# liuxinren456852/HiDeGS

Measured on AMD Instinct MI355X. Metric: binning-stage iters/sec at 2M Gaussians, 1920x1080 (scan + tile sort + ranges, the built part of the fwd+bwd iteration; the rasterizer fwd/bwd is not built: headline_metric, status), higher is better.
Workload: dtype u64/u32 (binning), f32 (distCUDA2, exchange, masked Adam)

## Files before the change

hidegs_amd/csrc/common.h:

```cpp
#pragma once
#include <hip/hip_runtime.h>
#include <stddef.h>
#include <stdint.h>

#include <string>

#include "../../include/hidegs.h"

namespace hidegs {

void set_error(const std::string& msg);
const std::string& last_error();

inline int fail(int code, const std::string& msg)
{
    set_error(msg);
    return code;
}

inline hipStream_t as_stream(void* s) { return reinterpret_cast<hipStream_t>(s); }

int check_launch(const char* stage, hipStream_t stream, int debug);

bool debug_enabled();

int queue_error(hipStream_t stream, int clear, uint32_t* flags);

uint32_t* async_error_slot(hipStream_t stream);
int take_async_error(const char* what, hipStream_t stream);
uint32_t take_async_bits(hipStream_t stream);

size_t sort_u64_scratch(long long n);
int sort_pairs_u64(void* scratch, size_t bytes, const uint64_t* ki, uint64_t* ko, const uint32_t* vi, uint32_t* vo,
                   long long n, int b, int e, hipStream_t s);

constexpr size_t kAlign = 256;
inline size_t align_up(size_t n) { return (n + kAlign - 1) & ~(kAlign - 1); }

struct Carver {
    char* base;
    size_t used = 0;
    explicit Carver(void* b) : base(static_cast<char*>(b)) {}
    template <typename T>
    T* take(size_t count)
    {
        T* p = reinterpret_cast<T*>(base ? base + used : nullptr);
        used += align_up(count * sizeof(T));
        return p;
    }
};

constexpr int kWave = 64;

__device__ __forceinline__ int lane_id() { return __lane_id(); }

__device__ __forceinline__ int xcd_swizzle(int b, int nb)
{
    const int per = nb / 8, rem = nb % 8, x = b % 8, k = b / 8;
    return (x < rem) ? x * (per + 1) + k : rem * (per + 1) + (x - rem) * per + k;
}

template <typename T>
__device__ __forceinline__ T wave_shfl_xor(T v, int m)
{
    return __shfl_xor(v, m, kWave);
}

__device__ __forceinline__ uint32_t wave_inclusive_scan_u32(uint32_t v)
{
    const int lane = lane_id(), rl = lane & 15;
    int x = (int)v, t;
    t = __builtin_amdgcn_mov_dpp(x, 0x111, 0xf, 0xf, false);
    if (rl >= 1) x += t;
    t = __builtin_amdgcn_mov_dpp(x, 0x112, 0xf, 0xf, false);
    if (rl >= 2) x += t;
    t = __builtin_amdgcn_mov_dpp(x, 0x114, 0xf, 0xf, false);
    if (rl >= 4) x += t;
    t = __builtin_amdgcn_mov_dpp(x, 0x118, 0xf, 0xf, false);
    if (rl >= 8) x += t;
    t = __builtin_amdgcn_mov_dpp(x, 0x142, 0xf, 0xf, false);
    if ((lane & 31) >= 16) x += t;
    t = __builtin_amdgcn_mov_dpp(x, 0x143, 0xf, 0xf, false);
    if (lane >= 32) x += t;
    return (uint32_t)x;
}

__device__ __forceinline__ float wave_max(float v)
{
#pragma unroll
    for (int m = 32; m >= 1; m >>= 1) v = fmaxf(v, __shfl_xor(v, m, kWave));
    return v;
}
__device__ __forceinline__ float wave_min(float v)
{
#pragma unroll
    for (int m = 32; m >= 1; m >>= 1) v = fminf(v, __shfl_xor(v, m, kWave));
    return v;
}
__device__ __forceinline__ float wave_sum(float v)
{
#pragma unroll
    for (int m = 32; m >= 1; m >>= 1) v += __shfl_xor(v, m, kWave);
    return v;
}
__device__ __forceinline__ uint32_t wave_sum_u32(uint32_t v)
{
#pragma unroll
    for (int m = 32; m >= 1; m >>= 1) v += __shfl_xor(v, m, kWave);
    return v;
}

}

namespace hidegs {

bool kernel_timing_enabled();
struct LaunchTimer {
    const char* name;
    hipStream_t stream;
    hipEvent_t start = nullptr, stop = nullptr;
    LaunchTimer(const char* n, hipStream_t s);
    ~LaunchTimer();
};

}

#define HIDEGS_LAUNCH(NAME, KERNEL, GRID, BLOCK, SHMEM, STREAM, ...)                        \
    do {                                                                                   \
        if (::hidegs::kernel_timing_enabled()) {                                           \
            ::hidegs::LaunchTimer _t(NAME, STREAM);                                        \
            hipLaunchKernelGGL(KERNEL, GRID, BLOCK, SHMEM, STREAM, __VA_ARGS__);           \
        } else {                                                                           \
            hipLaunchKernelGGL(KERNEL, GRID, BLOCK, SHMEM, STREAM, __VA_ARGS__);           \
        }                                                                                  \
    } while (0)
```

hidegs_amd/csrc/segment_forms.h:

```cpp
#pragma once

constexpr int kSegRun = 1024;
constexpr int kSegCap = 2 * kSegRun;
constexpr int kRunItems = kSegRun / kBlock;
constexpr int kSegItems = kSegCap / kBlock;

struct SegShared {
    uint32_t k[2][kSegRun];
    uint16_t i[2][kSegRun];
    uint32_t cnt[kWavesPerBlock][kRadix];
    uint32_t start[kRadix];
    uint32_t wave[kWavesPerBlock];
};

__device__ __forceinline__ int lds_radix_sort(SegShared& sh, const uint32_t n, const uint32_t diff)
{
    const int t = threadIdx.x, lane = lane_id(), wave = t / kWave;
    const uint32_t C = ((n + kBlock - 1) / kBlock) * kWave;
    const int rounds = (int)(C / kWave);
    const uint32_t w0 = wave * C;
    int cur = 0;
    for (int shift = 0; shift < 32; shift += kRadixBits) {
        const uint32_t vary = (diff >> shift) & (kRadix - 1);
        if (vary == 0) continue;
        for (int i = t; i < kWavesPerBlock * kRadix; i += kBlock) (&sh.cnt[0][0])[i] = 0;
        __syncthreads();
        uint32_t k[kRunItems], id[kRunItems], rank[kRunItems];
        bool ok[kRunItems];
#pragma unroll
        for (int q = 0; q < kRunItems; q++) {
            const uint32_t i = w0 + q * kWave + lane;
            ok[q] = q < rounds && i < n;
            k[q] = ok[q] ? sh.k[cur][i] : 0u;
            id[q] = ok[q] ? sh.i[cur][i] : 0u;
        }
        if (rounds == kRunItems) {
            wave_rank<uint32_t, kRunItems>(k, ok, shift, kRadix - 1, sh.cnt[wave], rank, vary);
        } else {
#pragma unroll
            for (int q = 0; q < kRunItems; q++) {
                if (q < rounds) {
                    uint32_t kk[1] = {k[q]}, rr[1];
                    bool oo[1] = {ok[q]};
                    wave_rank<uint32_t, 1>(kk, oo, shift, kRadix - 1, sh.cnt[wave], rr, vary);
                    rank[q] = rr[0];
                }
            }
        }
        __syncthreads();
        const uint32_t tot = digit_wave_prefix(sh.cnt);
        uint32_t dummy;
        sh.start[t] = block_exclusive_scan(tot, sh.wave, &dummy);
        __syncthreads();
#pragma unroll
        for (int q = 0; q < kRunItems; q++) {
            if (ok[q]) {
                const uint32_t dd = digit_of(k[q], shift, kRadix - 1);
                const uint32_t pos = sh.start[dd] + sh.cnt[wave][dd] + rank[q];
                sh.k[cur ^ 1][pos] = k[q];
                sh.i[cur ^ 1][pos] = id[q];
            }
        }
        __syncthreads();
        cur ^= 1;
    }
    return cur;
}

__device__ __forceinline__ uint32_t lds_rank(const uint32_t* a, uint32_t n, uint32_t key, bool inclusive)
{
    uint32_t lo = 0, len = n;
    while (len > 0) {
        const uint32_t half = len >> 1;
        const uint32_t v = a[lo + half];
        const bool go_right = inclusive ? (v <= key) : (v < key);
        lo = go_right ? lo + half + 1 : lo;
        len = go_right ? len - half - 1 : half;
    }
    return lo;
}

__device__ __forceinline__ void wave_and_or(uint32_t& a, uint32_t& o)
{
#pragma unroll
    for (int sh = 32; sh >= 1; sh >>= 1) {
        a &= __shfl_xor(a, sh, kWave);
        o |= __shfl_xor(o, sh, kWave);
    }
}

__device__ __forceinline__ void wave_min_max(uint32_t& lo, uint32_t& hi)
{
#pragma unroll
    for (int sh = 32; sh >= 1; sh >>= 1) {
        lo = min(lo, (uint32_t)__shfl_xor(lo, sh, kWave));
        hi = max(hi, (uint32_t)__shfl_xor(hi, sh, kWave));
    }
}

struct BigShared {
    uint32_t cnt[kWavesPerBlock][kRadix];
    uint32_t hist[kRadix];
    uint32_t run[kRadix];
    uint32_t aux[2][kRadix];
    uint32_t wave[kWavesPerBlock];
};

constexpr int kBigItems = 8;
constexpr int kBigStep = kBigItems * kBlock;
__device__ __forceinline__ void step_load(const uint64_t* sk, const uint32_t* sv, const uint32_t base,
                                          const uint32_t cnt, uint64_t (&k)[kBigItems], uint32_t (&v)[kBigItems])
{
    const uint32_t w0 = (threadIdx.x / kWave) * (kBigItems * kWave);
#pragma unroll
    for (int q = 0; q < kBigItems; q++) {
        const uint32_t i = w0 + q * kWave + lane_id();
        k[q] = i < cnt ? sk[base + i] : 0ull;
        v[q] = i < cnt ? sv[base + i] : 0u;
    }
}

template <bool Track = false>
__device__ __forceinline__ void step_scatter(const uint64_t (&k)[kBigItems], const uint32_t (&v)[kBigItems],
                                             const uint32_t cnt, uint64_t* dk, uint32_t* dv, const uint32_t dbase,
                                             const int shift, const uint32_t mask, const uint32_t lo,
                                             const uint32_t hi, BigShared& sh)
{
    const int t = threadIdx.x;
    const int lane = lane_id();
    const int wave = t / kWave;
    for (int i = t; i < kWavesPerBlock * kRadix; i += kBlock) (&sh.cnt[0][0])[i] = 0;
    __syncthreads();
    bool ok[kBigItems];
    uint32_t rank[kBigItems];
    const uint32_t w0 = wave * (kBigItems * kWave);
#pragma unroll
    for (int q = 0; q < kBigItems; q++) ok[q] = w0 + q * kWave + lane < cnt;
    wave_rank<uint64_t, kBigItems, true>(k, ok, shift, mask, sh.cnt[wave], rank, mask, dbase);
    __syncthreads();
    const uint32_t tot = digit_wave_prefix(sh.cnt);
    __syncthreads();
#pragma unroll
    for (int q = 0; q < kBigItems; q++) {
        if (ok[q]) {
            const uint32_t dd = (((uint32_t)k[q] - dbase) >> shift) & mask;
            const uint32_t dst = sh.run[dd] + sh.cnt[wave][dd] + rank[q];
            if (dst >= lo && dst < hi) {
                dk[dst] = k[q];
                dv[dst] = v[q];
            }
            if (Track) {
                atomicMin(&sh.aux[0][dd], (uint32_t)k[q]);
                atomicMax(&sh.aux[1][dd], (uint32_t)k[q]);
            }
        }
    }
    __syncthreads();
    sh.run[threadIdx.x] += tot;
    __syncthreads();
}

__device__ __forceinline__ void scatter_step(const uint64_t* sk, const uint32_t* sv, uint64_t* dk, uint32_t* dv,
                                             const uint32_t base, const uint32_t cnt, const uint32_t dbase,
                                             const int shift, const uint32_t mask, const uint32_t lo,
                                             const uint32_t hi, BigShared& sh)
{
    uint64_t k[kBigItems];
    uint32_t v[kBigItems];
    step_load(sk, sv, base, cnt, k, v);
    step_scatter(k, v, cnt, dk, dv, dbase, shift, mask, lo, hi, sh);
}

template <bool Track = false>
__device__ __forceinline__ void scatter_steps(const uint64_t* sk, const uint32_t* sv, uint64_t* dk, uint32_t* dv,
                                              const uint32_t base, const uint32_t cnt, const uint32_t dbase,
                                              const int shift, const uint32_t mask, const uint32_t lo,
                                              const uint32_t hi, BigShared& sh)
{
    uint64_t k[kBigItems], kn[kBigItems];
    uint32_t v[kBigItems], vn[kBigItems];
    step_load(sk, sv, base, cnt < (uint32_t)kBigStep ? cnt : (uint32_t)kBigStep, k, v);
    for (uint32_t b0 = 0; b0 < cnt; b0 += kBigStep) {
        const uint32_t c = cnt - b0 < (uint32_t)kBigStep ? cnt - b0 : (uint32_t)kBigStep;
        const uint32_t b1 = b0 + kBigStep;
        if (b1 < cnt) step_load(sk, sv, base + b1, cnt - b1 < (uint32_t)kBigStep ? cnt - b1 : (uint32_t)kBigStep, kn, vn);
        step_scatter<Track>(k, v, c, dk, dv, dbase, shift, mask, lo, hi, sh);
#pragma unroll
        for (int q = 0; q < kBigItems; q++) {
            k[q] = kn[q];
            v[q] = vn[q];
        }
    }
}

__device__ __forceinline__ void segment_sort_global(uint64_t* __restrict__ keys, uint32_t* __restrict__ vals,
                                                    uint64_t* __restrict__ alt_k, uint32_t* __restrict__ alt_v,
                                                    const uint32_t begin, const uint32_t m, BigShared& sh)
{
    const int t = threadIdx.x;
    for (int pass = 0; pass < 4; pass++) {
        const int shift = pass * kRadixBits;
        const uint64_t* sk = (pass & 1) ? alt_k : keys;
        const uint32_t* sv = (pass & 1) ? alt_v : vals;
        uint64_t* dk = (pass & 1) ? keys : alt_k;
        uint32_t* dv = (pass & 1) ? vals : alt_v;
        sh.hist[t] = 0;
        __syncthreads();
        for (uint32_t i = t; i < m; i += kBlock) atomicAdd(&sh.hist[digit_of(sk[begin + i], shift, kRadix - 1)], 1u);
        __syncthreads();
        uint32_t dummy;
        sh.run[t] = begin + block_exclusive_scan(sh.hist[t], sh.wave, &dummy);
        for (uint32_t c0 = 0; c0 < m; c0 += kBigStep)
            scatter_step(sk, sv, dk, dv, begin + c0, m - c0 < (uint32_t)kBigStep ? m - c0 : (uint32_t)kBigStep, 0u,
                         shift, kRadix - 1, begin, begin + m, sh);
    }
}

template <bool InPlace>
__device__ __forceinline__ void segment_sort_lsd(const uint64_t* __restrict__ src_k, const uint32_t* __restrict__ src_v,
                                                 uint64_t* __restrict__ dst_k, uint32_t* __restrict__ dst_v,
                                                 const uint32_t begin, const uint32_t m, const uint32_t diff,
                                                 SegShared& sh)
{
    uint64_t* dk = InPlace ? const_cast<uint64_t*>(src_k) : dst_k;
    uint32_t* dv = InPlace ? const_cast<uint32_t*>(src_v) : dst_v;
    const int t = threadIdx.x;
    const uint32_t na = m < (uint32_t)kSegRun ? m : (uint32_t)kSegRun, nb = m - na;
    uint32_t bk[kRunItems];
#pragma unroll
    for (int q = 0; q < kRunItems; q++) {
        const uint32_t i = t + q * kBlock;
        if (i < na) {
            sh.k[0][i] = (uint32_t)src_k[begin + i];
            sh.i[0][i] = i;
        }
        bk[q] = i < nb ? (uint32_t)src_k[begin + kSegRun + i] : 0u;
    }
    __syncthreads();
    const int ca = lds_radix_sort(sh, na, diff);

    uint32_t fk[kSegItems], fi[kSegItems], fp[kSegItems];
    bool fok[kSegItems];
    if (nb == 0) {
#pragma unroll
        for (int q = 0; q < kSegItems; q++) {
            const uint32_t i = t + q * kBlock;
            fok[q] = q < kRunItems && i < na;
            fp[q] = i;
            fk[q] = fok[q] ? sh.k[ca][i] : 0u;
            fi[q] = fok[q] ? sh.i[ca][i] : 0u;
        }
    } else {
        uint32_t ak[kRunItems], ai[kRunItems];
#pragma unroll
        for (int q = 0; q < kRunItems; q++) {
            ak[q] = sh.k[ca][t + q * kBlock];
            ai[q] = sh.i[ca][t + q * kBlock];
        }
        __syncthreads();
#pragma unroll
        for (int q = 0; q < kRunItems; q++) {
            const uint32_t i = t + q * kBlock;
            if (i < nb) {
                sh.k[0][i] = bk[q];
                sh.i[0][i] = kSegRun + i;
            }
        }
        __syncthreads();
        const int cb = lds_radix_sort(sh, nb, diff);
#pragma unroll
        for (int q = 0; q < kRunItems; q++) {
            sh.k[cb ^ 1][t + q * kBlock] = ak[q];
            sh.i[cb ^ 1][t + q * kBlock] = ai[q];
        }
        __syncthreads();
#pragma unroll
        for (int q = 0; q < kRunItems; q++) {
            const uint32_t i = t + q * kBlock;
            fok[q] = true;
            fk[q] = ak[q];
            fi[q] = ai[q];
            fp[q] = i + lds_rank(sh.k[cb], nb, ak[q], false);
            const uint32_t j = i;
            fok[kRunItems + q] = j < nb;
            fk[kRunItems + q] = fok[kRunItems + q] ? sh.k[cb][j] : 0u;
            fi[kRunItems + q] = fok[kRunItems + q] ? sh.i[cb][j] : 0u;
            fp[kRunItems + q] = fok[kRunItems + q] ? j + lds_rank(sh.k[cb ^ 1], kSegRun, fk[kRunItems + q], true) : 0u;
        }
    }
    uint32_t hi[kSegItems], v[kSegItems];
#pragma unroll
    for (int q = 0; q < kSegItems; q++) {
        if (fok[q]) {
            hi[q] = (uint32_t)(src_k[begin + fi[q]] >> 32);
            v[q] = src_v[begin + fi[q]];
        }
    }
    __syncthreads();
#pragma unroll
    for (int q = 0; q < kSegItems; q++) {
        if (fok[q]) {
            dk[begin + fp[q]] = ((uint64_t)hi[q] << 32) | fk[q];
            dv[begin + fp[q]] = v[q];
        }
    }
}

constexpr int kBucketBits = 10;
constexpr int kBuckets = 1 << kBucketBits;
constexpr int kMaxBucket = 128;
constexpr int kIndexBits = 11;
constexpr int kSegWaves = 7;

static_assert(kSegCap <= (1 << kIndexBits), "segment index must fit its field");

struct SegStats {
    uint32_t diff, lo;
    int shift, dbits;
};
__device__ __forceinline__ SegStats segment_stats(uint32_t a, uint32_t o, uint32_t lo, uint32_t hi, uint32_t* s0,
                                                  uint32_t* s1)
{
    const int lane = lane_id(), wave = threadIdx.x / kWave;
    wave_and_or(a, o);
    wave_min_max(lo, hi);
    if (lane == 0) {
        s0[wave] = a;
        s1[wave] = o;
    }
    __syncthreads();
    uint32_t aa = 0xffffffffu, oo = 0u;
#pragma unroll
    for (int w = 0; w < kWavesPerBlock; w++) {
        aa &= s0[w];
        oo |= s1[w];
    }
    __syncthreads();
    if (lane == 0) {
        s0[wave] = lo;
        s1[wave] = hi;
    }
    __syncthreads();
    uint32_t ll = 0xffffffffu, hh = 0u;
#pragma unroll
    for (int w = 0; w < kWavesPerBlock; w++) {
        ll = min(ll, s0[w]);
        hh = max(hh, s1[w]);
    }
    SegStats st;
    st.diff = aa ^ oo;
    st.lo = ll;
    const int nbits = hh > ll ? 32 - __builtin_clz(hh - ll) : 0;
    st.dbits = nbits < kBucketBits ? nbits : kBucketBits;
    st.shift = nbits - st.dbits;
    return st;
}


struct BucketShared {
    uint32_t comb[kSegCap];
    uint32_t start[kBuckets];
    uint32_t fill[kBuckets];
};
static_assert(sizeof(BucketShared) >= kSegCap * sizeof(uint64_t), "staging of the keys");
static_assert(sizeof(BucketShared) >= kSegRun * (sizeof(uint64_t) + sizeof(uint32_t)), "staging of a run");
static_assert(sizeof(BucketShared) >= kSegCap * 2 * sizeof(uint32_t), "compact staging of a segment");
```

hidegs_amd/csrc/segment_sort.h:

```cpp
#pragma once

union SegLds {
    SegShared lsd;
    BucketShared bucket;
    BigShared big;
    struct {
        BigShared big;
        EmitShared emit;
        uint32_t list[kBlock];
        uint32_t nlist;
    } queue;
};

union QueueLds {
    SegLds seg;
    WideShared wide;
};


template <bool Packed = false>
__device__ __forceinline__ void seg_load(const uint64_t* __restrict__ src_k, const uint32_t* __restrict__ src_v,
                                         const uint32_t begin, const uint32_t m, const uint32_t ref_hi,
                                         uint64_t (&k)[kSegItems], uint32_t (&v)[kSegItems], uint32_t& a, uint32_t& o,
                                         uint32_t& lo, uint32_t& hi, uint32_t& hd)
{
    const int t = threadIdx.x;
#pragma unroll
    for (int q = 0; q < kSegItems; q++) {
        const uint32_t i = t + q * kBlock;
        if (i < m) {
            if (Packed) {
                const uint2 rec = reinterpret_cast<const uint2*>(src_k)[begin + i];
                k[q] = ((uint64_t)ref_hi << 32) | rec.x;
                v[q] = rec.y;
            } else {
                k[q] = src_k[begin + i];
                v[q] = src_v[begin + i];
            }
            const uint32_t x = (uint32_t)k[q];
            a &= x;
            o |= x;
            lo = min(lo, x);
            hi = max(hi, x);
            hd |= (uint32_t)(k[q] >> 32) ^ ref_hi;
        }
    }
}

__device__ __forceinline__ void store_loaded(const uint64_t (&k)[kSegItems], const uint32_t (&v)[kSegItems],
                                             const uint32_t begin, const uint32_t m, uint64_t* dk, uint32_t* dv)
{
#pragma unroll
    for (int q = 0; q < kSegItems; q++) {
        const uint32_t i = threadIdx.x + q * kBlock;
        if (i < m) {
            dk[begin + i] = k[q];
            dv[begin + i] = v[q];
        }
    }
}

__device__ __forceinline__ uint32_t bucket_starts(const uint64_t (&k)[kSegItems], const uint32_t m,
                                                  const uint32_t base_lo, const int shift, const uint32_t hd,
                                                  BucketShared& sh, uint32_t* s_and, uint32_t* s_max,
                                                  uint32_t& mixed_hi)
{
    const int t = threadIdx.x, lane = lane_id(), wave = t / kWave;
#pragma unroll
    for (int q = 0; q < kSegItems; q++)
        if (t + q * kBlock < m) atomicAdd(&sh.fill[((uint32_t)k[q] - base_lo) >> shift], 1u);
    __syncthreads();
    uint32_t c[kBuckets / kBlock], sum = 0, mx = 0;
#pragma unroll
    for (int j = 0; j < kBuckets / kBlock; j++) {
        c[j] = sh.fill[t * (kBuckets / kBlock) + j];
        sum += c[j];
        mx = c[j] > mx ? c[j] : mx;
    }
    uint32_t dummy;
    uint32_t pre = block_exclusive_scan(sum, s_max, &dummy);
#pragma unroll
    for (int s = 32; s >= 1; s >>= 1) {
        const uint32_t y = __shfl_xor(mx, s, kWave);
        mx = y > mx ? y : mx;
    }
    const bool wave_hd = __ballot(hd != 0u) != 0ull;
    if (lane == 0) s_and[wave] = mx | (wave_hd ? 0x80000000u : 0u);
#pragma unroll
    for (int j = 0; j < kBuckets / kBlock; j++) {
        sh.start[t * (kBuckets / kBlock) + j] = pre;
        sh.fill[t * (kBuckets / kBlock) + j] = pre;
        pre += c[j];
    }
    __syncthreads();
    uint32_t fullest = 0;
    mixed_hi = 0;
#pragma unroll
    for (int w = 0; w < kWavesPerBlock; w++) {
        const uint32_t f = s_and[w] & 0x7fffffffu;
        fullest = f > fullest ? f : fullest;
        mixed_hi |= s_and[w] >> 31;
    }
    return fullest;
}

__device__ __forceinline__ void stage_compact(const uint64_t (&k)[kSegItems], const uint32_t (&v)[kSegItems],
                                              const uint32_t (&pos)[kSegItems], const uint32_t begin,
                                              const uint32_t m, const uint32_t ref_hi, BucketShared& sh, uint64_t* dk,
                                              uint32_t* dv)
{
    const int t = threadIdx.x;
    uint32_t* stage_lo = reinterpret_cast<uint32_t*>(&sh);
    uint32_t* stage_vv = stage_lo + kSegCap;
#pragma unroll
    for (int q = 0; q < kSegItems; q++) {
        if (t + q * kBlock < m) {
            stage_lo[pos[q]] = (uint32_t)k[q];
            stage_vv[pos[q]] = v[q];
        }
    }
    __syncthreads();
    const uint64_t khi = (uint64_t)ref_hi << 32;
#pragma unroll
    for (int q = 0; q < kSegItems; q++) {
        const uint32_t i = t + q * kBlock;
        if (i < m) {
            dk[begin + i] = khi | stage_lo[i];
            dv[begin + i] = stage_vv[i];
        }
    }
}

__device__ __forceinline__ void stage_pairs(const uint64_t (&k)[kSegItems], const uint32_t (&v)[kSegItems],
                                            const uint32_t (&pos)[kSegItems], const uint32_t begin, const uint32_t m,
                                            BucketShared& sh, uint64_t* dk, uint32_t* dv)
{
    const int t = threadIdx.x;
    uint64_t* stage_k = reinterpret_cast<uint64_t*>(&sh);
    uint32_t* stage_v = reinterpret_cast<uint32_t*>(stage_k + kSegRun);
    const bool together = m <= (uint32_t)kSegRun;
#pragma unroll
    for (int q = 0; q < kSegItems; q++) {
        if (t + q * kBlock < m) {
            stage_k[pos[q]] = k[q];
            if (together) stage_v[pos[q]] = v[q];
        }
    }
    __syncthreads();
#pragma unroll
    for (int q = 0; q < kSegItems; q++) {
        const uint32_t i = t + q * kBlock;
        if (i < m) {
            dk[begin + i] = stage_k[i];
            if (together) dv[begin + i] = stage_v[i];
        }
    }
    if (together) return;
    __syncthreads();
    stage_v = reinterpret_cast<uint32_t*>(&sh);
#pragma unroll
    for (int q = 0; q < kSegItems; q++)
        if (t + q * kBlock < m) stage_v[pos[q]] = v[q];
    __syncthreads();
#pragma unroll
    for (int q = 0; q < kSegItems; q++) {
        const uint32_t i = t + q * kBlock;
        if (i < m) dv[begin + i] = stage_v[i];
    }
}

template <bool InPlace>
__device__ __forceinline__ void sort_segment(const uint64_t* __restrict__ src_k, const uint32_t* __restrict__ src_v,
                                             uint64_t* __restrict__ dst_k, uint32_t* __restrict__ dst_v,
                                             const uint32_t begin, const uint32_t m, SegLds& lds, uint32_t* s_and,
                                             uint32_t* s_or, uint32_t* s_max)
{
    uint64_t* dk = InPlace ? const_cast<uint64_t*>(src_k) : dst_k;
    uint32_t* dv = InPlace ? const_cast<uint32_t*>(src_v) : dst_v;
    const int t = threadIdx.x;
    uint64_t k[kSegItems];
    uint32_t v[kSegItems];
    uint32_t a = 0xffffffffu, o = 0, lo = 0xffffffffu, hi = 0;
    const uint32_t ref_hi = m ? (uint32_t)(src_k[begin] >> 32) : 0u;
    uint32_t hd = 0;
    seg_load(src_k, src_v, begin, m, ref_hi, k, v, a, o, lo, hi, hd);
    BucketShared& sh = lds.bucket;
    for (int i = t; i < kBuckets; i += kBlock) sh.fill[i] = 0u;
    const SegStats st = segment_stats(a, o, lo, hi, s_and, s_or);
    const uint32_t diff = st.diff;
    if (diff == 0) {
        if (!InPlace) {
#pragma unroll
            for (int q = 0; q < kSegItems; q++) {
                const uint32_t i = t + q * kBlock;
                if (i < m) {
                    dk[begin + i] = k[q];
                    dv[begin + i] = v[q];
                }
            }
        }
        return;
    }
    const int shift = st.shift;
    uint32_t mixed_hi;
    const uint32_t fullest = bucket_starts(k, m, st.lo, shift, hd, sh, s_and, s_max, mixed_hi);
    if (fullest > (uint32_t)kMaxBucket || shift + kIndexBits > 32) {
        __syncthreads();
        segment_sort_lsd<InPlace>(src_k, src_v, dst_k, dst_v, begin, m, diff, lds.lsd);
        return;
    }
    const uint32_t base_lo = st.lo;
    const uint32_t lowmask = (uint32_t)((1ull << shift) - 1ull);
    uint32_t me[kSegItems];
    uint32_t bucket[kSegItems];
#pragma unroll
    for (int q = 0; q < kSegItems; q++) {
        const uint32_t i = t + q * kBlock;
        if (i < m) {
            const uint32_t x = (uint32_t)k[q] - base_lo;
            bucket[q] = x >> shift;
            me[q] = ((x & lowmask) << kIndexBits) | i;
            sh.comb[atomicAdd(&sh.fill[bucket[q]], 1u)] = me[q];
        }
    }
    __syncthreads();
    uint32_t pos[kSegItems];
#pragma unroll
    for (int q = 0; q < kSegItems; q++) {
        if (t + q * kBlock < m) {
            const uint32_t s0 = sh.start[bucket[q]], e0 = sh.fill[bucket[q]];
            uint32_t rank = 0;
            for (uint32_t j = s0; j < e0; j++) rank += sh.comb[j] < me[q] ? 1u : 0u;
            pos[q] = s0 + rank;
        }
    }
    __syncthreads();
    if (!mixed_hi) {
        stage_compact(k, v, pos, begin, m, ref_hi, sh, dk, dv);
        return;
    }
    stage_pairs(k, v, pos, begin, m, sh, dk, dv);
}

constexpr int kOpenLocal = 24576;
static_assert(kOpenLocal <= (int)kGroupChunks * kChunk, "open_local plans an ungrouped record (pending == chunks)");
constexpr int kScouts = HIDEGS_SCOUTS;
constexpr int kScoutItems = 32;
static_assert(kScouts == 0 || kBlock * kScoutItems <= kScouts * kBlock, "HIDEGS_SCOUTS: at least 32 scouts (or 0)");
__device__ __forceinline__ void open_local(const uint64_t* keys, const BigQueue& q, const uint32_t begin,
                                           const uint32_t m, BigShared& sh, EmitShared& e, uint32_t* s_and,
                                           uint32_t* s_or)
{
    const int t = threadIdx.x, lane = lane_id(), wave = t / kWave;
    uint32_t lo = 0xffffffffu, hi = 0u;
    for (uint32_t i0 = 0; i0 < m; i0 += kChunk) {
        uint32_t x[kChunk / kBlock];
#pragma unroll
        for (int u = 0; u < kChunk / kBlock; u++) {
            const uint32_t i = i0 + u * kBlock + t;
            x[u] = key_low(keys, begin + (i < m ? i : 0u));
        }
#pragma unroll
        for (int u = 0; u < kChunk / kBlock; u++) {
            lo = min(lo, x[u]);
            hi = max(hi, x[u]);
        }
    }
    wave_min_max(lo, hi);
    if (lane == 0) {
        s_and[wave] = lo;
        s_or[wave] = hi;
    }
    __syncthreads();
    for (int w = 0; w < kWavesPerBlock; w++) {
        lo = min(lo, s_and[w]);
        hi = max(hi, s_or[w]);
    }
    if (lo == hi) return;
    if (t == 0) {
        runs_begin(e);
        const uint4 r = record_run<false>(q, begin, m, 0u, true, lo, hi);
        e.run[0] = r;
        e.base = (r.x & 0xffu) == J_HIST ? q.rec[r.y].pool : ~0u;
        if (e.base == ~0u) add_run(e, r);
    }
    __syncthreads();
    const uint32_t pool = e.base, rec = e.run[0].y, chunks = (m + kChunk - 1) / kChunk;
    if (pool != ~0u) {
        int shift, bits;
        range_digit(lo, hi, shift, bits);
        const uint32_t mask = (1u << bits) - 1u;
        uint32_t* col = q.pool + pool + t;
        for (uint32_t c = 0; c < chunks; c++) {
            const uint32_t c0 = c * kChunk;
            col[c * kRadix] = chunk_hist(keys, begin + c0, m - c0 < (uint32_t)kChunk ? m - c0 : (uint32_t)kChunk,
                                         lo, shift, mask, sh);
        }
        __syncthreads();
        plan_scatter<false>(col, chunks, begin, sh);
        if (t == 0) {
            runs_begin(e);
            add_run(e, J_SCATTER, 0u, rec, 0u, chunks);
        }
    }
    emit_jobs(q, e);
}

constexpr int kExpandItems = 8;
__device__ __forceinline__ void expand_records(uint64_t* keys, uint32_t* vals, const uint32_t begin, const uint32_t m,
                                               const uint32_t seg)
{
    const uint2* recs = reinterpret_cast<const uint2*>(keys);
    const uint64_t khi = (uint64_t)seg << 32;
    for (uint32_t i0 = 0; i0 < m; i0 += kExpandItems * kBlock) {
        uint2 rec[kExpandItems];
#pragma unroll
        for (int u = 0; u < kExpandItems; u++) {
            const uint32_t i = i0 + u * kBlock + threadIdx.x;
            rec[u] = i < m ? recs[begin + i] : make_uint2(0u, 0u);
        }
#pragma unroll
        for (int u = 0; u < kExpandItems; u++) {
            const uint32_t i = i0 + u * kBlock + threadIdx.x;
            if (i < m) {
                keys[begin + i] = khi | rec[u].x;
                vals[begin + i] = rec[u].y;
            }
        }
    }
}

template <bool Packed>
__global__ __launch_bounds__(kBlock) __attribute__((amdgpu_waves_per_eu(kSegWaves))) void segment_sort_kernel(
    uint64_t* __restrict__ keys, uint32_t* __restrict__ vals, const uint32_t* __restrict__ starts,
    uint2* __restrict__ ranges_out, const int nseg, const BigQueue q)
{
    __shared__ __attribute__((aligned(16))) SegLds lds;
    __shared__ uint32_t s_and[kWavesPerBlock], s_or[kWavesPerBlock], s_max[kWavesPerBlock];
    if (kScouts > 0 && blockIdx.x < (unsigned)kScouts) {
        uint32_t* list = lds.queue.list;
        uint32_t carry = 0u;
        for (uint32_t s0 = 0; s0 < (uint32_t)nseg; s0 += kBlock * kScoutItems) {
            if (threadIdx.x == 0) lds.queue.nlist = 0u;
            uint32_t hot = 0u;
#pragma unroll 8
            for (int u = 0; u < kScoutItems; u++) {
                const uint32_t sg = s0 + (uint32_t)u * kBlock + threadIdx.x;
                if (sg < (uint32_t)nseg && starts[sg + 1] - starts[sg] > (uint32_t)kQueueMin) hot |= 1u << u;
            }
            uint32_t nhot;
            const uint32_t base = carry + block_exclusive_scan((uint32_t)__builtin_popcount(hot), s_max, &nhot);
            carry += nhot;
            if (nhot == 0u) continue;
            uint32_t ord = base;
            for (uint32_t h = hot; h; h &= h - 1u, ord++)
                if (ord % (uint32_t)kScouts == blockIdx.x)
                    list[atomicAdd(&lds.queue.nlist, 1u)] = s0 + (uint32_t)__builtin_ctz(h) * kBlock + threadIdx.x;
            __syncthreads();
            const uint32_t nl = lds.queue.nlist;
            for (uint32_t j = 0; j < nl; j++) {
                const uint32_t sg2 = list[j], b = starts[sg2], mm = starts[sg2 + 1] - b;
                if (HIDEGS_WIDE_SCOUTS && mm <= (uint32_t)kWideCap) {
                    if (threadIdx.x == 0) {
                        runs_begin(lds.queue.emit);
                        add_run(lds.queue.emit, J_WIDE, 0u, b, mm, 1u);
                    }
                    emit_jobs(q, lds.queue.emit);
                } else if (mm <= (uint32_t)kOpenLocal) {
                    open_local(keys, q, b, mm, lds.queue.big, lds.queue.emit, s_and, s_or);
                } else {
                    if (threadIdx.x == 0) {
                        runs_begin(lds.queue.emit);
                        add_run(lds.queue.emit, record_run(q, b, mm, 0u, false, 0u, 0u));
                    }
                    emit_jobs(q, lds.queue.emit);
                }
                __syncthreads();
            }
        }
        return;
    }
    const uint32_t seg = blockIdx.x - kScouts;
    const uint2 r = make_uint2(starts[seg], starts[seg + 1]);
    if (ranges_out && threadIdx.x == 0) ranges_out[seg] = r.y > r.x ? r : make_uint2(0u, 0u);
    const uint32_t begin = r.x, m = r.y - r.x;
    if (r.y <= r.x + 1) {
        if (Packed && r.y == r.x + 1) expand_records(keys, vals, begin, 1u, seg);
        return;
    }
    if (m > (uint32_t)kSegCap) {
        if (Packed) {
            expand_records(keys, vals, begin, m, seg);
            if (m <= (uint32_t)kQueueMin || kScouts == 0) __syncthreads();
        }
        if (m <= (uint32_t)kQueueMin) {
            segment_sort_global(keys, vals, q.alt_k, q.alt_v, begin, m, lds.big);
            return;
        }
        if (kScouts > 0) return;
        if (m <= (uint32_t)kOpenLocal) {
            open_local(keys, q, begin, m, lds.queue.big, lds.queue.emit, s_and, s_or);
            return;
        }
        if (threadIdx.x == 0) {
            runs_begin(lds.queue.emit);
            add_run(lds.queue.emit, record_run(q, begin, m, 0u, false, 0u, 0u));
        }
        emit_jobs(q, lds.queue.emit);
        return;
    }
    const int t = threadIdx.x;
    uint64_t k[kSegItems];
    uint32_t v[kSegItems];
    uint32_t a = 0xffffffffu, o = 0, lo = 0xffffffffu, hi = 0;
    const uint32_t ref_hi = Packed ? seg : (uint32_t)(keys[begin] >> 32);
    uint32_t hd = 0;
    seg_load<Packed>(keys, vals, begin, m, ref_hi, k, v, a, o, lo, hi, hd);
    BucketShared& sh = lds.bucket;
    for (int i = t; i < kBuckets; i += kBlock) sh.fill[i] = 0u;
    const SegStats st = segment_stats(a, o, lo, hi, s_and, s_or);
    const uint32_t diff = st.diff;
    if (diff == 0) {
        if (Packed) expand_records(keys, vals, begin, m, seg);
        return;
    }
    const int shift = st.shift;
    uint32_t mixed_hi;
    const uint32_t fullest = bucket_starts(k, m, st.lo, shift, hd, sh, s_and, s_max, mixed_hi);
    if (fullest > (uint32_t)kMaxBucket || shift + kIndexBits > 32) {
        if (Packed) store_loaded(k, v, begin, m, keys, vals);
        __syncthreads();
        segment_sort_lsd<true>(keys, vals, nullptr, nullptr, begin, m, diff, lds.lsd);
        return;
    }
    const uint32_t base_lo = st.lo;
    const uint32_t lowmask = (uint32_t)((1ull << shift) - 1ull);
    uint32_t me[kSegItems];
    uint32_t bucket[kSegItems];
#pragma unroll
    for (int q = 0; q < kSegItems; q++) {
        const uint32_t i = t + q * kBlock;
        if (i < m) {
            const uint32_t x = (uint32_t)k[q] - base_lo;
            bucket[q] = x >> shift;
            me[q] = ((x & lowmask) << kIndexBits) | i;
            sh.comb[atomicAdd(&sh.fill[bucket[q]], 1u)] = me[q];
        }
    }
    __syncthreads();
    uint32_t pos[kSegItems];
#pragma unroll
    for (int q = 0; q < kSegItems; q++) {
        if (t + q * kBlock < m) {
            const uint32_t s0 = sh.start[bucket[q]], e0 = sh.fill[bucket[q]];
            uint32_t rank = 0;
            for (uint32_t j = s0; j < e0; j++) rank += sh.comb[j] < me[q] ? 1u : 0u;
            pos[q] = s0 + rank;
        }
    }
    __syncthreads();
    if (Packed || !mixed_hi) {
        stage_compact(k, v, pos, begin, m, ref_hi, sh, keys, vals);
        return;
    }
    stage_pairs(k, v, pos, begin, m, sh, keys, vals);
}

__device__ __forceinline__ bool finish_phase(uint32_t& pending, uint32_t* s_flag)
{
    wave_stores_done();
    __syncthreads();
    if (threadIdx.x == 0) {
        release_lane();
        const bool last = __hip_atomic_fetch_add(&pending, 0xffffffffu, __ATOMIC_RELAXED, __HIP_MEMORY_SCOPE_AGENT) == 1u;
        if (last) acquire_lane();
        *s_flag = last;
    }
    __syncthreads();
    return *s_flag != 0;
}

__global__ __launch_bounds__(kBlock) void big_segment_kernel(uint64_t* __restrict__ keys, uint32_t* __restrict__ vals,
                                                             uint64_t* __restrict__ alt_k,
                                                             uint32_t* __restrict__ alt_v, const BigQueue q)
{
    __shared__ __attribute__((aligned(16))) QueueLds qlds;
    __shared__ uint32_t s_and[kWavesPerBlock], s_or[kWavesPerBlock], s_max[kWavesPerBlock];
    __shared__ uint4 s_job;
    __shared__ uint32_t s_flag;
    SegLds& lds = qlds.seg;
    const int t = threadIdx.x, lane = lane_id(), wave = t / kWave;
    BigShared& sh = lds.queue.big;
    EmitShared& e = lds.queue.emit;
    if (t == 0) s_flag = q_peek(&q.ctl[kCtlStride * Q_RESERVE]);
    __syncthreads();
    if (s_flag == 0) return;
#ifdef HIDEGS_QUEUE_TRACE
    unsigned long long t_claim = 0, t_got = 0;
    uint32_t t_index = 0;
#endif
    for (;;) {
        __syncthreads();
        if (t == 0) {
            const uint32_t i = __hip_atomic_fetch_add(&q.ctl[kCtlStride * Q_HEAD], 1u, __ATOMIC_RELAXED,
                                                      __HIP_MEMORY_SCOPE_AGENT);
#ifdef HIDEGS_QUEUE_TRACE
            t_claim = wall_clock64();
            t_index = i;
#endif
            uint4 job = make_uint4(J_EXIT, 0u, 0u, 0u);
            uint32_t polls = 0, backoff = 1;
            bool reserved = false;
            for (; polls < kMaxPolls; polls++) {
                if (i < q.job_cap && q_peek(&q.job[i].w) != 0u) {
                    acquire_lane();
                    job = q.job[i];
                    break;
                }
                if (!reserved) {
                    const uint32_t r0 = q_peek(&q.ctl[kCtlStride * Q_RESERVE]);
                    reserved = i < r0 && i < q.job_cap;
                    if (!reserved && q_peek(&q.ctl[kCtlStride * Q_DONE]) == r0) {
                        const uint32_t d = q_load(&q.ctl[kCtlStride * Q_DONE]);
                        const uint32_t r = q_load(&q.ctl[kCtlStride * Q_RESERVE]);
                        if (d == r && i >= r) break;
                    }
                }
                for (uint32_t k = 0; k < backoff; k++) __builtin_amdgcn_s_sleep(8);
                backoff = backoff < kBackoffMax ? 2u * backoff : kBackoffMax;
            }
            if (polls == kMaxPolls) q_flag(q, 4u);
            s_job = job;
#ifdef HIDEGS_QUEUE_TRACE
            t_got = wall_clock64();
#endif
        }
        __syncthreads();
        const uint4 job = s_job;
        const uint32_t type = job.x & 0xffu, src = job.x >> 8;
        if (type == J_EXIT) return;

        if (type == J_WIDE) {
            wide_sort(keys, vals, alt_k, alt_v, job.y, job.z, src, qlds.wide);
        } else if (type == J_SMALL) {
            if (src)
                sort_segment<false>(alt_k, alt_v, keys, vals, job.y, job.z, lds, s_and, s_or, s_max);
            else
                sort_segment<true>(keys, vals, nullptr, nullptr, job.y, job.z, lds, s_and, s_or, s_max);
        } else if (type == J_COPY) {
            for (uint32_t i = t; i < job.z; i += kBlock) {
                keys[job.y + i] = alt_k[job.y + i];
                vals[job.y + i] = alt_v[job.y + i];
            }
        } else if (type == J_GLOBAL) {
            if (src) {
                for (uint32_t i = t; i < job.z; i += kBlock) {
                    keys[job.y + i] = alt_k[job.y + i];
                    vals[job.y + i] = alt_v[job.y + i];
                }
                __syncthreads();
            }
            segment_sort_global(keys, vals, alt_k, alt_v, job.y, job.z, sh);
        } else {
            BigSeg& s = q.rec[job.y];
            const uint32_t c = job.z, begin = s.begin, m = s.m, chunks = s.chunks, csize = s.csize;
            const uint32_t c0 = c * csize, cnt = m - c0 < csize ? m - c0 : csize;
            const uint64_t* sk = s.src ? alt_k : keys;
            uint32_t* col = q.pool + s.pool + t;
            if (type == J_REDUCE) {
                uint32_t lo = 0xffffffffu, hi = 0u;
                for (uint32_t i0 = 0; i0 < cnt; i0 += kQueueIlp * kChunk) {
                    uint32_t x[kQueueIlp * kChunk / kBlock];
#pragma unroll
                    for (int u = 0; u < kQueueIlp * kChunk / kBlock; u++) {
                        const uint32_t i = i0 + t + u * kBlock;
                        x[u] = i < cnt ? (uint32_t)sk[begin + c0 + i] : 0xffffffffu;
                    }
#pragma unroll
                    for (int u = 0; u < kQueueIlp * kChunk / kBlock; u++) {
                        const uint32_t i = i0 + t + u * kBlock;
                        lo = min(lo, x[u]);
                        hi = i < cnt ? max(hi, x[u]) : hi;
                    }
                }
                wave_min_max(lo, hi);
                if (lane == 0) {
                    s_and[wave] = lo;
                    s_or[wave] = hi;
                }
                __syncthreads();
                if (t == 0) {
                    for (int w = 0; w < kWavesPerBlock; w++) {
                        lo = min(lo, s_and[w]);
                        hi = max(hi, s_or[w]);
                    }
                    __hip_atomic_fetch_min(&s.lo_bits, lo, __ATOMIC_RELAXED, __HIP_MEMORY_SCOPE_AGENT);
                    __hip_atomic_fetch_max(&s.hi_bits, hi, __ATOMIC_RELAXED, __HIP_MEMORY_SCOPE_AGENT);
                }
                if (finish_phase(s.pending, &s_flag)) {
                    if (t == 0) {
                        runs_begin(e);
                        const uint32_t rlo = q_load(&s.lo_bits), rhi = q_load(&s.hi_bits);
                        if (rlo == rhi) {
                            if (s.src) add_run(e, J_COPY, 1u, begin, m, (m + kChunk - 1) / kChunk);
                        } else {
                            set_digit(s, rlo, rhi);
                            s.pending = hist_countdown(q, s);
                            add_run(e, J_HIST, 0u, job.y, 0u, chunks);
                        }
                    }
                    emit_jobs(q, e);
                }
            } else if (type == J_HIST) {
                const int shift = (int)s.shift;
                const uint32_t mask = (1u << s.bits) - 1u;
                col[c * kRadix] = chunk_hist<kQueueIlp>(sk, begin + c0, cnt, s.lo, shift, mask, sh);
                const uint32_t ng = num_groups(chunks);
                bool last;
                if (ng) {
                    const uint32_t G = group_chunks(chunks), g = c / G, g0 = g * G;
                    last = finish_phase(q.pool[s.pool + (chunks + 4 + ng) * kRadix + g], &s_flag);
                    if (last) {
                        col[(chunks + 4 + g) * kRadix] = scan_column(col, g0, chunks - g0 < G ? chunks - g0 : G, 0u);
                        last = finish_phase(s.pending, &s_flag);
                    }
                } else {
                    last = finish_phase(s.pending, &s_flag);
                }
                if (last) {
                    plan_scatter(col, chunks, begin, sh);
                    if (t == 0) {
                        s.pending = chunks;
                        runs_begin(e);
                        add_run(e, J_SCATTER, 0u, job.y, 0u, chunks);
                    }
                    emit_jobs(q, e);
                }
            } else {
                const int shift = (int)s.shift;
                const uint32_t mask = (1u << s.bits) - 1u;
                const uint32_t dst = s.src ^ 1u;
                const uint32_t* sv = s.src ? alt_v : vals;
                uint64_t* dk = dst ? alt_k : keys;
                uint32_t* dv = dst ? alt_v : vals;
                const uint32_t ng = num_groups(chunks);
                sh.run[t] = col[c * kRadix] + (ng ? col[(chunks + 4 + c / group_chunks(chunks)) * kRadix] : 0u);
                sh.aux[0][t] = 0xffffffffu;
                sh.aux[1][t] = 0u;
                scatter_steps<true>(sk, sv, dk, dv, begin + c0, cnt, s.lo, shift, mask, begin, begin + m, sh);
                if (sh.aux[0][t] != 0xffffffffu || sh.aux[1][t] != 0u) {
                    __hip_atomic_fetch_min(&col[(chunks + 2) * kRadix], sh.aux[0][t], __ATOMIC_RELAXED,
                                           __HIP_MEMORY_SCOPE_AGENT);
                    __hip_atomic_fetch_max(&col[(chunks + 3) * kRadix], sh.aux[1][t], __ATOMIC_RELAXED,
                                           __HIP_MEMORY_SCOPE_AGENT);
                }
                if (finish_phase(s.pending, &s_flag)) {
                    cut_pieces(q, e, sh, col, chunks, begin, m, shift, dst);
                    emit_jobs(q, e);
                }
            }
        }
        __syncthreads();
        if (t == 0) __hip_atomic_fetch_add(&q.ctl[kCtlStride * Q_DONE], 1u, __ATOMIC_RELAXED, __HIP_MEMORY_SCOPE_AGENT);
#ifdef HIDEGS_QUEUE_TRACE
        if (t == 0) {
            const unsigned int slot = atomicAdd(&g_qtrace_n, 1u);
            if (slot < kQTraceCap) {
                const uint32_t last = (type == J_REDUCE || type == J_HIST || type == J_SCATTER) && s_flag ? 0x80u : 0u;
                g_qtrace[slot][0] = (unsigned long long)(type | last | (blockIdx.x << 8)) | ((unsigned long long)t_index << 32);
                g_qtrace[slot][1] = t_claim;
                g_qtrace[slot][2] = t_got;
                g_qtrace[slot][3] = wall_clock64();
            }
        }
#endif
    }
}

constexpr int kPieceBlocks = 256 * kPieceWaves;
__global__ __launch_bounds__(kBlock) __attribute__((amdgpu_waves_per_eu(kPieceWaves))) void piece_sort_kernel(
    uint64_t* __restrict__ keys, uint32_t* __restrict__ vals, const uint64_t* __restrict__ alt_k,
    const uint32_t* __restrict__ alt_v, const BigQueue q, uint32_t* async_err)
{
    __shared__ __attribute__((aligned(16))) SegLds lds;
    __shared__ uint32_t s_and[kWavesPerBlock], s_or[kWavesPerBlock], s_max[kWavesPerBlock];
    if (async_err && blockIdx.x == 0 && threadIdx.x == 0) {
        const uint32_t err = q_peek(&q.ctl[kCtlStride * Q_ERROR]);
        if (err) {
            const uint32_t old = __hip_atomic_load(async_err, __ATOMIC_RELAXED, __HIP_MEMORY_SCOPE_SYSTEM);
            __hip_atomic_store(async_err, old | err, __ATOMIC_RELAXED, __HIP_MEMORY_SCOPE_SYSTEM);
        }
    }
    const uint32_t np = min(q.ctl[kCtlStride * Q_NPIECE], q.piece_cap);
    for (uint32_t p = blockIdx.x; p < np; p += gridDim.x) {
        const uint2 e = q.piece[p];
        const uint32_t m = e.y & 0x7fffffffu;
        if (e.y >> 31)
            sort_segment<false>(alt_k, alt_v, keys, vals, e.x, m, lds, s_and, s_or, s_max);
        else
            sort_segment<true>(keys, vals, nullptr, nullptr, e.x, m, lds, s_and, s_or, s_max);
        __syncthreads();
    }
}
```

Measured before the change: 6258.

## Trim segment sort register pressure and use DPP wave reductions

Wave min/max/and/or reductions now use DPP row ops plus readlane instead of xor shuffles. The AND/OR diff computation is taken out of the load loop and is computed only on the LSD fallback path, so the common path only tracks the min/max range. The Packed variant skips the high-word check and gets a higher waves-per-EU target. Bucket and rank temporaries are recomputed rather than held in arrays, and staging uses packed uint2 LDS stores. The aim is fewer VGPRs and less cross-lane work for higher occupancy. The cost is an extra block reduction with a barrier on the fallback path, plus recomputing the key math.

```diff
diff --git a/hidegs_amd/csrc/common.h b/hidegs_amd/csrc/common.h
--- a/hidegs_amd/csrc/common.h
+++ b/hidegs_amd/csrc/common.h
@@ -85,6 +85,36 @@
     return (uint32_t)x;
 }
 
+#define HIDEGS_DPP_SELF(x, ctrl, rows) ((uint32_t)__builtin_amdgcn_update_dpp((int)(x), (int)(x), ctrl, rows, 0xf, false))
+template <typename Op>
+__device__ __forceinline__ uint32_t wave_reduce_u32(uint32_t x, Op op)
+{
+    x = op(x, HIDEGS_DPP_SELF(x, 0x111, 0xf));
+    x = op(x, HIDEGS_DPP_SELF(x, 0x112, 0xf));
+    x = op(x, HIDEGS_DPP_SELF(x, 0x114, 0xf));
+    x = op(x, HIDEGS_DPP_SELF(x, 0x118, 0xf));
+    x = op(x, HIDEGS_DPP_SELF(x, 0x142, 0xa));
+    x = op(x, HIDEGS_DPP_SELF(x, 0x143, 0xc));
+    return (uint32_t)__builtin_amdgcn_readlane((int)x, kWave - 1);
+}
+#undef HIDEGS_DPP_SELF
+struct OpMinU32 {
+    __device__ __forceinline__ uint32_t operator()(uint32_t a, uint32_t b) const { return a < b ? a : b; }
+};
+struct OpMaxU32 {
+    __device__ __forceinline__ uint32_t operator()(uint32_t a, uint32_t b) const { return a > b ? a : b; }
+};
+struct OpAndU32 {
+    __device__ __forceinline__ uint32_t operator()(uint32_t a, uint32_t b) const { return a & b; }
+};
+struct OpOrU32 {
+    __device__ __forceinline__ uint32_t operator()(uint32_t a, uint32_t b) const { return a | b; }
+};
+__device__ __forceinline__ uint32_t wave_min_u32(uint32_t v) { return wave_reduce_u32(v, OpMinU32()); }
+__device__ __forceinline__ uint32_t wave_max_u32(uint32_t v) { return wave_reduce_u32(v, OpMaxU32()); }
+__device__ __forceinline__ uint32_t wave_and_u32(uint32_t v) { return wave_reduce_u32(v, OpAndU32()); }
+__device__ __forceinline__ uint32_t wave_or_u32(uint32_t v) { return wave_reduce_u32(v, OpOrU32()); }
+
 __device__ __forceinline__ float wave_max(float v)
 {
 #pragma unroll
diff --git a/hidegs_amd/csrc/segment_forms.h b/hidegs_amd/csrc/segment_forms.h
--- a/hidegs_amd/csrc/segment_forms.h
+++ b/hidegs_amd/csrc/segment_forms.h
@@ -82,20 +82,14 @@
 
 __device__ __forceinline__ void wave_and_or(uint32_t& a, uint32_t& o)
 {
-#pragma unroll
-    for (int sh = 32; sh >= 1; sh >>= 1) {
-        a &= __shfl_xor(a, sh, kWave);
-        o |= __shfl_xor(o, sh, kWave);
-    }
+    a = wave_and_u32(a);
+    o = wave_or_u32(o);
 }
 
 __device__ __forceinline__ void wave_min_max(uint32_t& lo, uint32_t& hi)
 {
-#pragma unroll
-    for (int sh = 32; sh >= 1; sh >>= 1) {
-        lo = min(lo, (uint32_t)__shfl_xor(lo, sh, kWave));
-        hi = max(hi, (uint32_t)__shfl_xor(hi, sh, kWave));
-    }
+    lo = wave_min_u32(lo);
+    hi = wave_max_u32(hi);
 }
 
 struct BigShared {
@@ -311,6 +305,7 @@
 constexpr int kMaxBucket = 128;
 constexpr int kIndexBits = 11;
 constexpr int kSegWaves = 7;
+constexpr int kSegWavesPacked = 8;
 
 static_assert(kSegCap <= (1 << kIndexBits), "segment index must fit its field");
 
@@ -354,6 +349,59 @@
     st.dbits = nbits < kBucketBits ? nbits : kBucketBits;
     st.shift = nbits - st.dbits;
     return st;
+}
+
+struct SegRange {
+    uint32_t lo, hi;
+    int shift;
+};
+__device__ __forceinline__ SegRange segment_range(uint32_t lo, uint32_t hi, uint32_t* s0, uint32_t* s1)
+{
+    const int lane = lane_id(), wave = threadIdx.x / kWave;
+    wave_min_max(lo, hi);
+    if (lane == 0) {
+        s0[wave] = lo;
+        s1[wave] = hi;
+    }
+    __syncthreads();
+    SegRange r;
+    r.lo = 0xffffffffu;
+    r.hi = 0u;
+#pragma unroll
+    for (int w = 0; w < kWavesPerBlock; w++) {
+        r.lo = min(r.lo, s0[w]);
+        r.hi = max(r.hi, s1[w]);
+    }
+    const int nbits = r.hi > r.lo ? 32 - __builtin_clz(r.hi - r.lo) : 0;
+    r.shift = nbits - (nbits < kBucketBits ? nbits : kBucketBits);
+    return r;
+}
+
+__device__ __forceinline__ uint32_t segment_diff(const uint64_t (&k)[kSegItems], const uint32_t m, uint32_t* s0,
+                                                 uint32_t* s1)
+{
+    const int lane = lane_id(), wave = threadIdx.x / kWave;
+    uint32_t a = 0xffffffffu, o = 0u;
+#pragma unroll
+    for (int q = 0; q < kSegItems; q++) {
+        if (threadIdx.x + q * kBlock < m) {
+            a &= (uint32_t)k[q];
+            o |= (uint32_t)k[q];
+        }
+    }
+    wave_and_or(a, o);
+    if (lane == 0) {
+        s0[wave] = a;
+        s1[wave] = o;
+    }
+    __syncthreads();
+    uint32_t aa = 0xffffffffu, oo = 0u;
+#pragma unroll
+    for (int w = 0; w < kWavesPerBlock; w++) {
+        aa &= s0[w];
+        oo |= s1[w];
+    }
+    return aa ^ oo;
 }
 
 
diff --git a/hidegs_amd/csrc/segment_sort.h b/hidegs_amd/csrc/segment_sort.h
--- a/hidegs_amd/csrc/segment_sort.h
+++ b/hidegs_amd/csrc/segment_sort.h
@@ -21,8 +21,8 @@
 template <bool Packed = false>
 __device__ __forceinline__ void seg_load(const uint64_t* __restrict__ src_k, const uint32_t* __restrict__ src_v,
                                          const uint32_t begin, const uint32_t m, const uint32_t ref_hi,
-                                         uint64_t (&k)[kSegItems], uint32_t (&v)[kSegItems], uint32_t& a, uint32_t& o,
-                                         uint32_t& lo, uint32_t& hi, uint32_t& hd)
+                                         uint64_t (&k)[kSegItems], uint32_t (&v)[kSegItems], uint32_t& lo, uint32_t& hi,
+                                         uint32_t& hd)
 {
     const int t = threadIdx.x;
 #pragma unroll
@@ -38,11 +38,9 @@
                 v[q] = src_v[begin + i];
             }
             const uint32_t x = (uint32_t)k[q];
-            a &= x;
-            o |= x;
             lo = min(lo, x);
             hi = max(hi, x);
-            hd |= (uint32_t)(k[q] >> 32) ^ ref_hi;
+            if (!Packed) hd |= (uint32_t)(k[q] >> 32) ^ ref_hi;
         }
     }
 }
@@ -60,6 +58,7 @@
     }
 }
 
+template <bool OneHi = false>
 __device__ __forceinline__ uint32_t bucket_starts(const uint64_t (&k)[kSegItems], const uint32_t m,
                                                   const uint32_t base_lo, const int shift, const uint32_t hd,
                                                   BucketShared& sh, uint32_t* s_and, uint32_t* s_max,
@@ -79,13 +78,13 @@
     }
     uint32_t dummy;
     uint32_t pre = block_exclusive_scan(sum, s_max, &dummy);
-#pragma unroll
-    for (int s = 32; s >= 1; s >>= 1) {
-        const uint32_t y = __shfl_xor(mx, s, kWave);
-        mx = y > mx ? y : mx;
-    }
-    const bool wave_hd = __ballot(hd != 0u) != 0ull;
-    if (lane == 0) s_and[wave] = mx | (wave_hd ? 0x80000000u : 0u);
+    mx = wave_max_u32(mx);
+    if (OneHi) {
+        if (lane == 0) s_and[wave] = mx;
+    } else {
+        const bool wave_hd = __ballot(hd != 0u) != 0ull;
+        if (lane == 0) s_and[wave] = mx | (wave_hd ? 0x80000000u : 0u);
+    }
 #pragma unroll
     for (int j = 0; j < kBuckets / kBlock; j++) {
         sh.start[t * (kBuckets / kBlock) + j] = pre;
@@ -97,9 +96,9 @@
     mixed_hi = 0;
 #pragma unroll
     for (int w = 0; w < kWavesPerBlock; w++) {
-        const uint32_t f = s_and[w] & 0x7fffffffu;
+        const uint32_t f = OneHi ? s_and[w] : s_and[w] & 0x7fffffffu;
         fullest = f > fullest ? f : fullest;
-        mixed_hi |= s_and[w] >> 31;
+        if (!OneHi) mixed_hi |= s_and[w] >> 31;
     }
     return fullest;
 }
@@ -110,23 +109,19 @@
                                               uint32_t* dv)
 {
     const int t = threadIdx.x;
-    uint32_t* stage_lo = reinterpret_cast<uint32_t*>(&sh);
-    uint32_t* stage_vv = stage_lo + kSegCap;
-#pragma unroll
-    for (int q = 0; q < kSegItems; q++) {
-        if (t + q * kBlock < m) {
-            stage_lo[pos[q]] = (uint32_t)k[q];
-            stage_vv[pos[q]] = v[q];
-        }
-    }
+    uint2* stage = reinterpret_cast<uint2*>(&sh);
+#pragma unroll
+    for (int q = 0; q < kSegItems; q++)
+        if (t + q * kBlock < m) stage[pos[q]] = make_uint2((uint32_t)k[q], v[q]);
     __syncthreads();
     const uint64_t khi = (uint64_t)ref_hi << 32;
 #pragma unroll
     for (int q = 0; q < kSegItems; q++) {
         const uint32_t i = t + q * kBlock;
         if (i < m) {
-            dk[begin + i] = khi | stage_lo[i];
-            dv[begin + i] = stage_vv[i];
+            const uint2 rec = stage[i];
+            dk[begin + i] = khi | rec.x;
+            dv[begin + i] = rec.y;
         }
     }
 }
@@ -180,15 +175,14 @@
     const int t = threadIdx.x;
     uint64_t k[kSegItems];
     uint32_t v[kSegItems];
-    uint32_t a = 0xffffffffu, o = 0, lo = 0xffffffffu, hi = 0;
+    uint32_t lo = 0xffffffffu, hi = 0;
     const uint32_t ref_hi = m ? (uint32_t)(src_k[begin] >> 32) : 0u;
     uint32_t hd = 0;
-    seg_load(src_k, src_v, begin, m, ref_hi, k, v, a, o, lo, hi, hd);
+    seg_load(src_k, src_v, begin, m, ref_hi, k, v, lo, hi, hd);
     BucketShared& sh = lds.bucket;
     for (int i = t; i < kBuckets; i += kBlock) sh.fill[i] = 0u;
-    const SegStats st = segment_stats(a, o, lo, hi, s_and, s_or);
-    const uint32_t diff = st.diff;
-    if (diff == 0) {
+    const SegRange st = segment_range(lo, hi, s_and, s_or);
+    if (st.lo == st.hi) {
         if (!InPlace) {
 #pragma unroll
             for (int q = 0; q < kSegItems; q++) {
@@ -205,7 +199,7 @@
     uint32_t mixed_hi;
     const uint32_t fullest = bucket_starts(k, m, st.lo, shift, hd, sh, s_and, s_max, mixed_hi);
     if (fullest > (uint32_t)kMaxBucket || shift + kIndexBits > 32) {
-        __syncthreads();
+        const uint32_t diff = segment_diff(k, m, s_max, s_or);
         segment_sort_lsd<InPlace>(src_k, src_v, dst_k, dst_v, begin, m, diff, lds.lsd);
         return;
     }
@@ -331,9 +325,9 @@
 }
 
 template <bool Packed>
-__global__ __launch_bounds__(kBlock) __attribute__((amdgpu_waves_per_eu(kSegWaves))) void segment_sort_kernel(
-    uint64_t* __restrict__ keys, uint32_t* __restrict__ vals, const uint32_t* __restrict__ starts,
-    uint2* __restrict__ ranges_out, const int nseg, const BigQueue q)
+__global__ __launch_bounds__(kBlock) __attribute__((amdgpu_waves_per_eu(Packed ? kSegWavesPacked : kSegWaves)))
+void segment_sort_kernel(uint64_t* __restrict__ keys, uint32_t* __restrict__ vals, const uint32_t* __restrict__ starts,
+                         uint2* __restrict__ ranges_out, const int nseg, const BigQueue q)
 {
     __shared__ __attribute__((aligned(16))) SegLds lds;
     __shared__ uint32_t s_and[kWavesPerBlock], s_or[kWavesPerBlock], s_max[kWavesPerBlock];
@@ -412,49 +406,49 @@
     const int t = threadIdx.x;
     uint64_t k[kSegItems];
     uint32_t v[kSegItems];
-    uint32_t a = 0xffffffffu, o = 0, lo = 0xffffffffu, hi = 0;
+    uint32_t lo = 0xffffffffu, hi = 0;
     const uint32_t ref_hi = Packed ? seg : (uint32_t)(keys[begin] >> 32);
     uint32_t hd = 0;
-    seg_load<Packed>(keys, vals, begin, m, ref_hi, k, v, a, o, lo, hi, hd);
+    seg_load<Packed>(keys, vals, begin, m, ref_hi, k, v, lo, hi, hd);
     BucketShared& sh = lds.bucket;
     for (int i = t; i < kBuckets; i += kBlock) sh.fill[i] = 0u;
-    const SegStats st = segment_stats(a, o, lo, hi, s_and, s_or);
-    const uint32_t diff = st.diff;
-    if (diff == 0) {
+    const SegRange st = segment_range(lo, hi, s_and, s_or);
+    if (st.lo == st.hi) {
         if (Packed) expand_records(keys, vals, begin, m, seg);
         return;
     }
     const int shift = st.shift;
     uint32_t mixed_hi;
-    const uint32_t fullest = bucket_starts(k, m, st.lo, shift, hd, sh, s_and, s_max, mixed_hi);
+    const uint32_t fullest = bucket_starts<Packed>(k, m, st.lo, shift, hd, sh, s_and, s_max, mixed_hi);
     if (fullest > (uint32_t)kMaxBucket || shift + kIndexBits > 32) {
         if (Packed) store_loaded(k, v, begin, m, keys, vals);
-        __syncthreads();
+        const uint32_t diff = segment_diff(k, m, s_max, s_or);
         segment_sort_lsd<true>(keys, vals, nullptr, nullptr, begin, m, diff, lds.lsd);
         return;
     }
     const uint32_t base_lo = st.lo;
     const uint32_t lowmask = (uint32_t)((1ull << shift) - 1ull);
-    uint32_t me[kSegItems];
-    uint32_t bucket[kSegItems];
 #pragma unroll
     for (int q = 0; q < kSegItems; q++) {
         const uint32_t i = t + q * kBlock;
         if (i < m) {
             const uint32_t x = (uint32_t)k[q] - base_lo;
-            bucket[q] = x >> shift;
-            me[q] = ((x & lowmask) << kIndexBits) | i;
-            sh.comb[atomicAdd(&sh.fill[bucket[q]], 1u)] = me[q];
+            sh.comb[atomicAdd(&sh.fill[x >> shift], 1u)] = ((x & lowmask) << kIndexBits) | i;
         }
     }
     __syncthreads();
     uint32_t pos[kSegItems];
 #pragma unroll
     for (int q = 0; q < kSegItems; q++) {
-        if (t + q * kBlock < m) {
-            const uint32_t s0 = sh.start[bucket[q]], e0 = sh.fill[bucket[q]];
+        const uint32_t i = t + q * kBlock;
+        if (i < m) {
+            uint32_t x = (uint32_t)k[q];
+            asm volatile("" : "+v"(x));
+            x -= base_lo;
+            const uint32_t b = x >> shift, me = ((x & lowmask) << kIndexBits) | i;
+            const uint32_t s0 = sh.start[b], e0 = sh.fill[b];
             uint32_t rank = 0;
-            for (uint32_t j = s0; j < e0; j++) rank += sh.comb[j] < me[q] ? 1u : 0u;
+            for (uint32_t j = s0; j < e0; j++) rank += sh.comb[j] < me ? 1u : 0u;
             pos[q] = s0 + rank;
         }
     }
```

After: 6473 (median of 6 runs). 1.03x the previous value.
